# lunarlab-gatech/SLIDE_SLAM

Hardware: AMD Instinct MI355X
Metric: pose-graph updates/sec + ms/Gauss-Newton iter, 8-robot 10k-landmark graph (higher is better)
Workload: dtype f64

## Files before the change

slide_slam_amd/csrc/graph_dev.hpp:

```cpp
#pragma once
#include <stdint.h>

namespace sl {

enum { VT_POSE = 0, VT_POINT = 1, VT_CUBE = 2, VT_CYL = 3 };
enum { FT_BR = 2, FT_CUBE = 3, FT_CYL = 4 };

constexpr int NB = 64;

__host__ __device__ inline int lm_dim(int t) { return t == VT_POINT ? 3 : (t == VT_CUBE ? 9 : 7); }
__host__ __device__ inline int lf_rows(int t) { return t == FT_BR ? 3 : (t == FT_CUBE ? 9 : 7); }
__host__ __device__ inline int lf_jsize(int t) { return t == FT_BR ? 30 : (t == FT_CUBE ? 144 : 98); }
__host__ __device__ inline int lf_esize(int t) { return t == FT_BR ? 42 : (t == FT_CUBE ? 114 : 90); }

struct GraphDev {
  int P, L;
  double* pose_val;
  double* pose_delta;
  double* pose_est;
  int* lm_type;
  double* lm_val;
  double* lm_delta;
  double* lm_est;
  int n_prior;
  int* pr_pose; double* pr_z; double* pr_sigma;
  double* pr_r;
  int n_between;
  int* bt_i; int* bt_j; double* bt_z; double* bt_sigma;
  double* bt_r; double* bt_J0;
  int n_ghost;
  int* gh_pose; int* gh_slot; int* gh_first;
  double* gh_z; double* gh_sigma;
  double* gh_r; double* gh_J;
  int n_gslots; double* ghost_val; int* gslot_pose;
  int n_lf;
  int n_nbr;
  int* lf_type; int* lf_pose; int* lf_lm; int* lf_slot;
  int* lf_nbr;
  int64_t* lf_joff; int64_t* lf_eoff;
  double* br_z;
  double* cu_z; double* cu_sigma;
  double* cy_z;
  double* jbuf;
  double* ebuf;
  int* lm_ptr; int* lm_fids;
  int* pose_ptr; int* pose_fids;
  int* pose_lms;
  long long* pose_ed;
  int* pose_bt_ptr; int* pose_bt;
  unsigned* pose_adj; int adj_words;
  double* lm_Hinv;
  double* lm_g;
  double* lm_Hacc;
  double* lm_t;
  int n_slots;
  int* sh_lid;
  int* sh_owner;
  double* pose_H;
  double* pose_g;
  double* S;
  int ld;
  int T;
  double* Ld;
  double* Winv;
  double* yv;
  double* dp;
  int* chol_ctr;
  const int* prof;
  const int* first;
  int prof_ver;
  int schur_split;
  double* S0;
  int save_S0;
  double* pcg;
  const int* lm_slot;
  double* pcg_scal;
  double pcg_tol2;
  int arrow;
  int nbr;
  const int* lm_bord;
  const int* seg_tab;
  double* bord;
  int ldb;
  double* bord0;
  const int* pose_sep;
  int nsep;
  int nsep_dim;
  const int* gh_bord;
  const int* lm_first;
  int pose0;
  int col0;
  const int* sp_idx;
  const long long* sp_pairs;
  int sp_w;
  int* status;
  int chart;
  double relin_thr;
  double bearing_sigma, cyl_sigma, numdiff_delta;
};

struct RobustDev {
  double* bt_sigma0;
  double* bt_w; double* bt_s2;
  int* bt_kind;
  double* gh_sigma0;
  double* gh_w; double* gh_s2;
  int kind;
  int mask;
  double param;
};

struct ObsLossDev {
  double* lf_w; double* lf_s2;
  int kind;
  int mask;
  double param;
};

}
```

slide_slam_amd/csrc/kernels.hpp:

```cpp
#pragma once
#include <hip/hip_runtime.h>
#include <stdint.h>

#include "graph_dev.hpp"
#include "sl_math.hpp"

namespace sl {

void init_solver_kernels();
void launch_relin(const GraphDev& G, hipStream_t s);
void launch_linearize(const GraphDev& G, const ObsLossDev& O, hipStream_t s);
void launch_observation_weights(const GraphDev& G, const ObsLossDev& O, bool robust, int n, double* out2n, hipStream_t s);
void launch_observation_weights_batched(const GraphDev* d, const ObsLossDev* dO, bool robust, const int* off, const int* cnt, int n, double* out2n,
                                        hipStream_t s);
void launch_robust_reweight(const GraphDev& G, const RobustDev& R, hipStream_t s);
void launch_closure_weights(const GraphDev& G, const RobustDev& R, const int* idx, int n, double* out2n, hipStream_t s);
void launch_robust_reweight_batched(const GraphDev* d, const RobustDev* dR, const GraphDev* h, int n, hipStream_t s);
void launch_closure_weights_batched(const GraphDev* d, const RobustDev* dR, const int* ent2, int n, double* out2n, hipStream_t s);
void launch_landmark(const GraphDev& G, int mode, hipStream_t s);
void launch_pose(const GraphDev& G, hipStream_t s);
void launch_schur(const GraphDev& G, hipStream_t s);
void launch_backsub(const GraphDev& G, int mode, hipStream_t s);
void launch_shared_pack(const GraphDev& G, int what, double* buf, hipStream_t s);
void launch_shared_unpack(const GraphDev& G, int what, const double* buf, hipStream_t s);
// ... 192 lines not shown
  }
  return lo;
}
struct TriSeg { int tm0, td0, ntd; };
void launch_tri_match_seg(bool emit, const double* sd, const double* sx, const int* rowoff, const TriSeg* segs, int n_seg, int n_rows, double thr,
                          int* counts, const long long* offs, const long long* base, double* P1, double* P2, hipStream_t s);
void launch_seg_scan64(const int* cnt, const int* segoff, int n_seg, long long* out, long long* totals, hipStream_t s);
void launch_seg_scan_rowptr(const int* cnt, const int* segoff, int n_seg, int* rowptr, long long* totals, hipStream_t s);
struct ClqSolve {
  const int* rowptr; const int* col; const double* val; int n;
  const double* u0;
  double *u, *unew, *g, *gnew, *Mu, *Cu;
  double tol_u, tol_F, beta, eps;
  int maxin, maxol, maxls, rescale;
  double* out;
};
void launch_clq_solve_batch(const ClqSolve* d_jobs, int n_jobs, hipStream_t s);
bool launch_clq_solve_coop(const ClqSolve& A, double* priv, int* bar2, int n_wg, hipStream_t s);
void launch_clq_csr_count(const double* Mup, int n, int* rowcnt, hipStream_t s);
void launch_clq_csr_fill(const double* Mup, int n, const int* rowptr, int* col, double* val, hipStream_t s);
void launch_clq_solve(const int* rowptr, const int* col, const double* val, int n, const double* u0, double* work6n, double tol_u, double tol_F,
                      double beta, double eps, int maxin, int maxol, int maxls, int rescale, double* out4, hipStream_t s);
void launch_clipper_affinity(const double* D1, const double* D2, int dim, const int32_t* A, int m, double sigma, double eps,
                             double mindist, double affinityeps, double* M, hipStream_t s);
template <int DIM>
__device__ __forceinline__ double clipper_pair_score(int i0, int i1, int j0, int j1, const double* pi1, const double* pj1, const double* pi2,
                                                     const double* pj2, int dim, double sigma, double eps, double mindist, double affinityeps) {
  double out = 0.0;
  if (i0 != j0 && i1 != j1) {
    const int nd = DIM > 0 ? DIM : dim;
    double s1 = 0, s2 = 0;
    for (int k = 0; k < nd; ++k) {
      s1 += (pi1[k] - pj1[k]) * (pi1[k] - pj1[k]);
      s2 += (pi2[k] - pj2[k]) * (pi2[k] - pj2[k]);
    }
    const double l1 = sqrt(s1), l2 = sqrt(s2);
    if (!(mindist > 0 && (l1 < mindist || l2 < mindist))) {
      const double c = fabs(l1 - l2);
      const double scr = (c < eps) ? exp(-0.5 * c * c / (sigma * sigma)) : 0.0;
      if (scr > affinityeps) out = scr;
    }
  }
  return out;
}
void launch_affinity_gather(const double* D1, const double* D2, int dim, const int32_t* A, int m, double* P1, double* P2, hipStream_t s);
void launch_affinity_csr(bool emit, const double* D1, const double* D2, const double* P1, const double* P2, int dim, const int32_t* A, int m,
                         double sigma, double eps, double mindist, double affinityeps, int* rowcnt, const int* rowptr, int* col, double* val,
                         hipStream_t s);
void launch_affinity_csr_seg(bool emit, const double* P1, const double* P2, const int* aoff, int n_seg, int n_rows, double sigma, double eps,
                             double mindist, double affinityeps, int* rowcnt, const int* rowptr, const long long* nnz0, int* col, double* val,
                             hipStream_t s);
void launch_clq_pack_u(const double* work, const int* aoff, int n_seg, int n_rows, double* U, hipStream_t s);

constexpr int CLOSURE_PRE = 36;
struct ClosureScore { double gate, sigma, affinityeps, odom2[6]; };
__host__ __device__ __forceinline__ double closure_pair_score(const double* __restrict__ pre_i, const double* __restrict__ pre_j, const double* __restrict__ s2i,
                                                              const double* __restrict__ s2j, double legs, const ClosureScore& P) {
  const SE3 E = compose(compose(from12(pre_i), from12(pre_j + 12)), from12(pre_i + 24));
  double e[6];
  se3_log(E, e);
  double q = 0.0;
#pragma unroll
  for (int c = 0; c < 6; ++c) q += e[c] * e[c] / (s2i[c] + s2j[c] + legs * P.odom2[c]);
  const double d = sqrt(q);
  const double scr = d < P.gate ? exp(-0.5 * d * d / (P.sigma * P.sigma)) : 0.0;
  return scr > P.affinityeps ? scr : 0.0;
}
__host__ __device__ __forceinline__ void closure_prepare_one(const SE3& F, const SE3& T, const SE3& z, double* __restrict__ pre) {
  const SE3 U = compose(z, inverse(T));
  to12(U, pre);
  to12(inverse(compose(F, U)), pre + 12);
  to12(F, pre + 24);
}
void launch_closure_prepare(const double* fpose12, const double* tpose12, const int32_t* fslot, const int32_t* tslot, const double* z12, int n,
                            double* pre, hipStream_t s);
void launch_closure_csr_seg(bool emit, const double* pre, const double* sig2, const unsigned long long* idx2, const int* goff, int n_seg,
                            int n_rows, const ClosureScore& P, int* rowcnt, const int* rowptr, const long long* nnz0, int* col, double* val,
                            hipStream_t s);

constexpr int GATE_OUT = 43;
void launch_closure_gate_lin(const double* pose_est, const int32_t* fslot, const int32_t* tslot, const double* z12, const double* sigma6, int n,
                             int chart, const int* prow, double* B, int nT, double* r6, hipStream_t s);
void launch_pair_identity(const int32_t* aslot, const int32_t* bslot, int n, const int* prow, double* B, int nT, hipStream_t s);
struct JointPoseTab { const double* est[JSIG_ROBOTS_MAX]; const int* prow[JSIG_ROBOTS_MAX]; long long off[JSIG_ROBOTS_MAX]; int chart[JSIG_ROBOTS_MAX]; };
void launch_joint_closure_gate_lin(const JointPoseTab* tab, const int4* ends, const double* z12, const double* sigma6, int n, double* B,
                                   size_t ld, double* r6, hipStream_t s);
void launch_joint_pair_identity(const JointPoseTab* tab, const int4* ends, int n, double* B, size_t ld, hipStream_t s);
void launch_gram_sub(double* M, const double* Mneg, size_t n, hipStream_t s);
void launch_closure_gate_finish(const double* M, const double* r6, int n, double* out, int* flag, hipStream_t s);

constexpr int OBS_GATE_OUT = 91;
void launch_obs_gate_lin(const GraphDev& G, int type, const int32_t* pid, const int32_t* lid, const double* z15, const double* sg9, int n,
                         double* B, int nT, double* r9, double* G0, hipStream_t s);
void launch_joint_obs_gate_lin(const GraphDev* Gs, const JointPoseTab* tab, int type, const int4* ends, const long long* sep_row, const double* z15,
                               const double* sg9, int n, double* B, size_t ld, double* r9, double* G0, hipStream_t s);
void launch_obs_gate_finish(int m, const double* M, const double* G0, const double* r9, int n, double* out, int* flag, hipStream_t s);

}
```

slide_slam_amd/csrc/pcg_kernels.hip:

```cpp
#include <hip/hip_runtime.h>

#include "graph_dev.hpp"
#include "kernels.hpp"

namespace sl {

enum { PV_R = 0, PV_U = 1, PV_W = 2, PV_P = 3, PV_S = 4, PV_X = 5, PV_Y = 6, PV_COUNT = 7 };
__device__ __forceinline__ double* pvec(const GraphDev& G, int i) { return G.pcg + (size_t)i * G.T * NB; }

__global__ __launch_bounds__(256) void k_pcg_init(const GraphDev* __restrict__ Gs) {
  const GraphDev G = Gs[blockIdx.z];
  const int i = blockIdx.x * 256 + threadIdx.x, nT = G.T * NB;
  if (i >= nT) return;
  pvec(G, PV_R)[i] = i < 6 * G.P ? -G.pose_g[i] : 0.0;
  pvec(G, PV_U)[i] = G.dp[i];
  pvec(G, PV_X)[i] = 0.0;
  pvec(G, PV_P)[i] = 0.0;
  pvec(G, PV_S)[i] = 0.0;
  if (i < 8) G.pcg_scal[i] = 0.0;
}

struct PcgBufs { double* p[8]; };

__device__ __forceinline__ void pcg_tl_body(const GraphDev& G, const PcgBufs& B, int blk, int vec) {
  const int wave = threadIdx.x >> 6, lane = threadIdx.x & 63;
  const int sidx = blk * 4 + wave;
  if (sidx >= G.n_slots) return;
  double* out = B.p[blockIdx.z] + 9 * (size_t)sidx;
  const int l = G.sh_lid[sidx];
  if (l < 0) {
    if (lane < 9) out[lane] = 0.0;
    return;
  }
  const double* v = pvec(G, vec);
  const int D = lm_dim(G.lm_type[l]);
  double rhs[9];
#pragma unroll
  for (int k = 0; k < 9; ++k) rhs[k] = 0.0;
  for (int q = G.lm_ptr[l] + lane; q < G.lm_ptr[l + 1]; q += 64) {
    const int f = G.lm_fids[q];
    const double* E = G.ebuf + G.lf_eoff[f];
    const double* d = v + 6 * (size_t)G.lf_pose[f];
    double dd[6];
#pragma unroll
    for (int a = 0; a < 6; ++a) dd[a] = d[a];
#pragma unroll
    for (int k = 0; k < 9; ++k) {
      if (k < D) {
        double s = 0.0;
#pragma unroll
        for (int a = 0; a < 6; ++a) s += E[a * D + k] * dd[a];
        rhs[k] += s;
      }
    }
  }
#pragma unroll
  for (int k = 0; k < 9; ++k) {
#pragma unroll
    for (int m = 32; m >= 1; m >>= 1) rhs[k] += __shfl_xor(rhs[k], m);
  }
  if (lane == 0) {
#pragma unroll
    for (int k = 0; k < 9; ++k) {
      G.lm_t[9 * (size_t)l + k] = rhs[k];
      out[k] = rhs[k];
    }
  }
}

__device__ __forceinline__ void pcg_symv_body(const GraphDev& G, int bi, int vin, int vout, int in_lds) {
  if (bi >= G.T) return;
  extern __shared__ double xs_lds[];
  __shared__ double red[4][NB];
  __shared__ double redt[NB][5];
  const int tid = threadIdx.x, row = tid & 63, cp = tid >> 6;
  const double* x = pvec(G, vin);
  const double* S0 = G.S0;
  const int ld = G.ld, nT = G.T * NB;
  if (in_lds) {
    for (int i = tid; i < nT; i += 256) xs_lds[i] = x[i];
    __syncthreads();
  }
  const double* xs = in_lds ? xs_lds : x;
  double acc = 0.0;
  {
    double ta[16], tb[16];
    const double* tp0 = S0 + (size_t)(16 * cp) * ld + (size_t)bi * NB + row;
    const int jf = G.first ? G.first[bi] : 0;
    if (jf < bi) {
      const double* tp = tp0 + (size_t)(jf * NB) * ld;
#pragma unroll
      for (int r = 0; r < 16; ++r) ta[r] = tp[(size_t)r * ld];
    }
    for (int j = jf; j < bi; j += 2) {
      if (j + 1 < bi) {
        const double* tp = tp0 + (size_t)((j + 1) * NB) * ld;
#pragma unroll
        for (int r = 0; r < 16; ++r) tb[r] = tp[(size_t)r * ld];
      }
      {
        const double* xj = xs + j * NB + 16 * cp;
#pragma unroll
        for (int r = 0; r < 16; ++r) acc += ta[r] * xj[r];
      }
      if (j + 2 < bi) {
        const double* tp = tp0 + (size_t)((j + 2) * NB) * ld;
#pragma unroll
        for (int r = 0; r < 16; ++r) ta[r] = tp[(size_t)r * ld];
      }
      if (j + 1 < bi) {
        const double* xj = xs + (j + 1) * NB + 16 * cp;
#pragma unroll
        for (int r = 0; r < 16; ++r) acc += tb[r] * xj[r];
      }
    }
  }
  {
    const double* tp = S0 + (size_t)(bi * NB) * ld + (size_t)bi * NB;
    const double* xj = xs + bi * NB;
#pragma unroll
    for (int r = 0; r < 16; ++r) {
      const int c = 16 * cp + r;
      const double v = c <= row ? tp[(size_t)c * ld + row] : tp[(size_t)row * ld + c];
      acc += v * xj[c];
    }
  }
  red[cp][row] = acc;
  const int col = tid >> 2, part = tid & 3;
  double acct = 0.0;
  {
    double ta[16], tb[16];
    const double* tp0 = S0 + (size_t)(bi * NB + col) * ld + 16 * part;
    const int j0 = bi + 1, T = G.prof ? G.prof[bi] + 1 : G.T;
    if (j0 < T) {
#pragma unroll
      for (int r = 0; r < 16; ++r) ta[r] = tp0[(size_t)j0 * NB + r];
    }
    for (int j = j0; j < T; j += 2) {
      if (j + 1 < T) {
#pragma unroll
        for (int r = 0; r < 16; ++r) tb[r] = tp0[(size_t)(j + 1) * NB + r];
      }
      {
        const double* xj = xs + j * NB + 16 * part;
#pragma unroll
        for (int r = 0; r < 16; ++r) acct += ta[r] * xj[r];
      }
      if (j + 2 < T) {
#pragma unroll
        for (int r = 0; r < 16; ++r) ta[r] = tp0[(size_t)(j + 2) * NB + r];
      }
      if (j + 1 < T) {
        const double* xj = xs + (j + 1) * NB + 16 * part;
#pragma unroll
        for (int r = 0; r < 16; ++r) acct += tb[r] * xj[r];
      }
    }
  }
  redt[col][part] = acct;
  __syncthreads();
  if (tid < NB) {
    const double a = (red[0][tid] + red[1][tid]) + (red[2][tid] + red[3][tid]);
    const double b = (redt[tid][0] + redt[tid][1]) + (redt[tid][2] + redt[tid][3]);
    pvec(G, vout)[(size_t)bi * NB + tid] = a + b;
  }
}

__global__ __launch_bounds__(256) void k_pcg_tl_symv(const GraphDev* __restrict__ Gs, PcgBufs B, int vec, int vout, int n_row_blocks, int in_lds) {
  const GraphDev G = Gs[blockIdx.z];
  if ((int)blockIdx.x < n_row_blocks) pcg_symv_body(G, blockIdx.x, vec, vout, in_lds);
  else pcg_tl_body(G, B, (int)blockIdx.x - n_row_blocks, vec);
}

__global__ __launch_bounds__(256) void k_pcg_cross(const GraphDev* __restrict__ Gs, PcgBufs B, int vout, int nsum) {
  const GraphDev G = Gs[blockIdx.z];
  const int wave = threadIdx.x >> 6, lane = threadIdx.x & 63;
  const int p = blockIdx.x * 4 + wave;
  if (p >= G.P) return;
  double y[6];
#pragma unroll
  for (int a = 0; a < 6; ++a) y[a] = 0.0;
  for (int q = G.pose_ptr[p] + lane; q < G.pose_ptr[p + 1]; q += 64) {
    const int l = G.pose_lms[q];
    const int sl = G.lm_slot[l];
    if (sl < 0) continue;
    const long long ed = G.pose_ed[q];
    const int D = (int)(ed & 15);
    const double* town = G.lm_t + 9 * (size_t)l;
    double cc[9];
#pragma unroll
    for (int k = 0; k < 9; ++k) cc[k] = 0.0;
    if (nsum > 1) {
#pragma unroll
      for (int k = 0; k < 9; ++k) {
        if (k < D) {
          double t[8];
#pragma unroll
          for (int r = 0; r < 8; ++r) t[r] = r < nsum ? B.p[r][9 * (size_t)sl + k] : 0.0;
          double acc = 0.0;
#pragma unroll
          for (int r = 0; r < 8; ++r)
            if (r < nsum) acc += t[r];
          cc[k] = acc;
        }
      }
    } else {
      const double* tsum = B.p[blockIdx.z] + 9 * (size_t)sl;
#pragma unroll
      for (int k = 0; k < 9; ++k) cc[k] = k < D ? tsum[k] : 0.0;
    }
#pragma unroll
    for (int k = 0; k < 9; ++k) cc[k] = k < D ? cc[k] - town[k] : 0.0;
    const double* F = G.ebuf + (ed >> 4) + 6 * D;
#pragma unroll
    for (int a = 0; a < 6; ++a) {
      double s = 0.0;
#pragma unroll
      for (int k = 0; k < 9; ++k)
        if (k < D) s += F[a * D + k] * cc[k];
      y[a] += s;
    }
  }
#pragma unroll
  for (int a = 0; a < 6; ++a) {
#pragma unroll
    for (int m = 32; m >= 1; m >>= 1) y[a] += __shfl_xor(y[a], m);
  }
  if (lane < 6) {
    double v = 0.0;
#pragma unroll
    for (int a = 0; a < 6; ++a) v = lane == a ? y[a] : v;
    pvec(G, vout)[6 * (size_t)p + lane] -= v;
  }
}

__global__ __launch_bounds__(256) void k_pcg_dots(const GraphDev* __restrict__ Gs, PcgBufs B) {
  const GraphDev G = Gs[blockIdx.z];
  __shared__ double sh[2][256];
  const int tid = threadIdx.x, nT = G.T * NB;
  const double* r = pvec(G, PV_R);
  const double* u = pvec(G, PV_U);
  const double* w = pvec(G, PV_W);
  double a = 0.0, b = 0.0;
  for (int i = tid; i < nT; i += 256) {
    const double ui = u[i];
    a += r[i] * ui;
    b += w[i] * ui;
  }
  sh[0][tid] = a;
  sh[1][tid] = b;
  __syncthreads();
  for (int st = 128; st > 0; st >>= 1) {
    if (tid < st) { sh[0][tid] += sh[0][tid + st]; sh[1][tid] += sh[1][tid + st]; }
// ... 105 lines not shown
```

slide_slam_amd/csrc/solver_kernels.hip:

```cpp
#include <hip/hip_runtime.h>
#include <algorithm>
#include <cstring>

#include "graph_dev.hpp"
#include "kernels.hpp"
#include "sl_math.hpp"

namespace sl {

struct BufPtrs { double* p[8]; };

__device__ inline void pose_retract12(const double* in12, const double* d6, int chart, double* out12) {
  to12(retract(from12(in12), d6, chart), out12);
}
__device__ inline void lm_retract(int type, const double* in, const double* d, int chart, double* out) {
  if (type == VT_POINT) {
    out[0] = in[0] + d[0]; out[1] = in[1] + d[1]; out[2] = in[2] + d[2];
  } else if (type == VT_CUBE) {
    pose_retract12(in, d, chart, out);
    out[12] = in[12] + d[6]; out[13] = in[13] + d[7]; out[14] = in[14] + d[8];
  } else {
    out[3] = in[3] + d[0]; out[4] = in[4] + d[1]; out[5] = in[5] + d[2];
    out[0] = in[0] + d[3]; out[1] = in[1] + d[4]; out[2] = in[2] + d[5];
    out[6] = in[6] + d[6];
// ... 214 lines not shown
#pragma unroll
        for (int k = 0; k < 3; ++k) { s += Dm[3 * r + k] * Q.a[3 * k + j]; u += Dm[3 * r + k] * X.R.a[3 * j + k]; }
        Jp[6 * r + j] = sc(s * w);
        Jp[6 * r + 3 + j] = sc(-Dm[3 * r + j] * w);
        Jl[3 * r + j] = sc(u * w);
      }
  } else if (type == FT_CUBE) {
    const double* z = G.cu_z + 15 * (size_t)slot;
    const double* sg = G.cu_sigma + 9 * (size_t)slot;
    const SE3 C = from12(lv);
    double dX[6], dC[6], cs[3];
#pragma unroll
    for (int k = 0; k < 6; ++k) { dX[k] = (col == k) ? d : 0.0; dC[k] = (col == 6 + k) ? d : 0.0; }
#pragma unroll
    for (int k = 0; k < 3; ++k) cs[k] = lv[12 + k] + ((col == 12 + k) ? d : 0.0);
    double e[9];
    cube_err(retract(X, dX, G.chart), retract(C, dC, G.chart), cs, z, e);
    if constexpr (ROBUST) {
      double s2 = 0.0;
#pragma unroll
      for (int i = 0; i < 9; ++i) { const double q = __shfl(e[i], 30, 32) * (1.0 / sg[i]); s2 += q * q; }
      sq = obs_loss_scale(O, FT_CUBE, f, s2, j == 30);
    }
#pragma unroll
    for (int i = 0; i < 9; ++i) {
      const double hx = __shfl(e[i], 30, 32), eo = __shfl_xor(e[i], 1, 32), w = 1.0 / sg[i];
      if (j == 30) out[i] = sc(hx * w);
      if ((j & 1) == 0 && col < 15) {
        const double v = sc(((e[i] - hx) - (eo - hx)) * fac * w);
        if (col < 6) out[9 + 6 * i + col] = v;
        else out[63 + 9 * i + col - 6] = v;
      }
    }
  } else {
    const double* z = G.cy_z + 7 * (size_t)slot;
    const double w = 1.0 / G.cyl_sigma;
    const int jl = col - 6;
    const int vi = jl < 0 ? -1 : (jl < 3 ? jl + 3 : (jl < 6 ? jl - 3 : (jl == 6 ? 6 : -1)));
    double dX[6], q[7];
#pragma unroll
    for (int k = 0; k < 6; ++k) dX[k] = (col == k) ? d : 0.0;
#pragma unroll
    for (int k = 0; k < 7; ++k) q[k] = lv[k] + ((vi == k) ? d : 0.0);
    double e[7];
    cyl_err(retract(X, dX, G.chart), q, z, e);
    if constexpr (ROBUST) {
      double s2 = 0.0;
#pragma unroll
      for (int i = 0; i < 7; ++i) { const double q = __shfl(e[i], 30, 32) * w; s2 += q * q; }
      sq = obs_loss_scale(O, FT_CYL, f, s2, j == 30);
    }
#pragma unroll
    for (int i = 0; i < 7; ++i) {
      const double hx = __shfl(e[i], 30, 32), eo = __shfl_xor(e[i], 1, 32);
      if (j == 30) out[i] = sc(hx * w);
      if ((j & 1) == 0 && col < 13) {
        const double v = sc(((e[i] - hx) - (eo - hx)) * fac * w);
        if (col < 6) out[7 + 6 * i + col] = v;
        else out[49 + 7 * i + jl] = v;
      }
    }
  }
}
__global__ __launch_bounds__(256) void k_lin_lf(GraphDev G, int nb0, int nb1) {
  if ((int)blockIdx.x < nb0) k_lin_pose_factors_body(G, blockIdx.x * 256 + threadIdx.x);
  else k_lin_lf_body<false>(G, ObsLossDev{}, nb1, (int)blockIdx.x - nb0);
}
__global__ __launch_bounds__(256) void k_lin_lf_robust(GraphDev G, ObsLossDev O, int nb0, int nb1) {
  if ((int)blockIdx.x < nb0) k_lin_pose_factors_body(G, blockIdx.x * 256 + threadIdx.x);
  else k_lin_lf_body<true>(G, O, nb1, (int)blockIdx.x - nb0);
}
__global__ __launch_bounds__(256) void k_lin_lf_b(const GraphDev* __restrict__ Gs, int nb0, int nb1) {
  if ((int)blockIdx.x < nb0) k_lin_pose_factors_body(Gs[blockIdx.z], blockIdx.x * 256 + threadIdx.x);
  else k_lin_lf_body<false>(Gs[blockIdx.z], ObsLossDev{}, nb1, (int)blockIdx.x - nb0);
}
__global__ __launch_bounds__(256) void k_lin_lf_robust_b(const GraphDev* __restrict__ Gs, const ObsLossDev* __restrict__ Os, int nb0, int nb1) {
  if ((int)blockIdx.x < nb0) k_lin_pose_factors_body(Gs[blockIdx.z], blockIdx.x * 256 + threadIdx.x);
  else k_lin_lf_body<true>(Gs[blockIdx.z], Os[blockIdx.z], nb1, (int)blockIdx.x - nb0);
}

__shared__ double lm_hs[4][96];
constexpr int LM_RED_MAX = 24;
__shared__ double lm_red[4][54 * LM_RED_MAX];

template <int D, int MODE>
__device__ inline void landmark_wave(const GraphDev& G, int l, int lane) {
  constexpr int NH = D * (D + 1) / 2;
  double h[NH], g[D];
#pragma unroll
  for (int i = 0; i < NH; ++i) h[i] = 0.0;
#pragma unroll
  for (int i = 0; i < D; ++i) g[i] = 0.0;
  const int f0 = G.lm_ptr[l], nf = G.lm_ptr[l + 1] - f0;
  double* acc = G.lm_Hacc + 54 * (size_t)l;
  if (MODE == 2) {
#pragma unroll
    for (int i = 0; i < NH; ++i) h[i] = acc[i];
#pragma unroll
    for (int i = 0; i < D; ++i) g[i] = acc[45 + i];
  }
  for (int q = lane; MODE != 2 && q < nf; q += 64) {
    const int f = G.lm_fids[f0 + q];
    const double* rec = G.jbuf + G.lf_joff[f];
    const double* Jl = rec + D + 6 * D;
#pragma unroll
    for (int k = 0; k < D; ++k) {
      double row[D];
#pragma unroll
      for (int a = 0; a < D; ++a) row[a] = Jl[D * k + a];
      const double rk = rec[k];
#pragma unroll
      for (int a = 0; a < D; ++a) {
        g[a] += row[a] * rk;
#pragma unroll
        for (int c = 0; c <= a; ++c) h[a * (a + 1) / 2 + c] += row[a] * row[c];
      }
    }
  }
  if (MODE != 2) {
    if (MODE == 3) {
      double* red = lm_red[threadIdx.x >> 6];
      const int nl = nf < 64 ? nf : 64;
      double tot = 0.0;
      for (int base = 0; base < nl; base += LM_RED_MAX) {
        const int cnt = nl - base < LM_RED_MAX ? nl - base : LM_RED_MAX;
        if (lane >= base && lane < base + cnt) {
#pragma unroll
          for (int i = 0; i < NH; ++i) red[i * LM_RED_MAX + lane - base] = h[i];
#pragma unroll
          for (int i = 0; i < D; ++i) red[(NH + i) * LM_RED_MAX + lane - base] = g[i];
        }
        __builtin_amdgcn_wave_barrier();
        __builtin_amdgcn_s_waitcnt(0xc07f);
        if (lane < NH + D)
          for (int q = 0; q < cnt; ++q) tot += red[lane * LM_RED_MAX + q];
        __builtin_amdgcn_wave_barrier();
        __builtin_amdgcn_s_waitcnt(0xc07f);
      }
      if (lane < NH + D) red[lane] = tot;
      __builtin_amdgcn_wave_barrier();
      __builtin_amdgcn_s_waitcnt(0xc07f);
#pragma unroll
      for (int i = 0; i < NH; ++i) h[i] = red[i];
#pragma unroll
      for (int i = 0; i < D; ++i) g[i] = red[NH + i];
    } else {
#pragma unroll
      for (int off = 32; off > 0; off >>= 1) {
#pragma unroll
        for (int i = 0; i < NH; ++i) h[i] += __shfl_xor(h[i], off);
#pragma unroll
        for (int i = 0; i < D; ++i) g[i] += __shfl_xor(g[i], off);
      }
    }
  }
  if (MODE == 1 || MODE == 3) {
    if (lane == 0) {
#pragma unroll
      for (int i = 0; i < NH; ++i) acc[i] = h[i];
#pragma unroll
      for (int i = 0; i < D; ++i) acc[45 + i] = g[i];
    }
    if (MODE == 1) return;
  }
  double* Hinv = G.lm_Hinv + 81 * (size_t)l;
  double* gout = G.lm_g + 9 * (size_t)l;
// ... 1 lines not shown
#pragma unroll
    for (int a = 0; a < D; ++a) gout[a] = g[a];
  }
  const bool sep = (MODE == 2 || MODE == 3) && G.arrow && G.lm_slot && G.lm_slot[l] >= 0;
  if (nf == 0 && (MODE == 0 || MODE == 3)) {
    if (lane == 0) {
#pragma unroll
      for (int i = 0; i < D * D; ++i) Hinv[i] = 0.0;
    }
    return;
  }
  double Cm[D][D];
  bool ok = true;
#pragma unroll
  for (int j = 0; j < D; ++j) {
    double s = h[j * (j + 1) / 2 + j];
#pragma unroll
    for (int k = 0; k < j; ++k) s -= Cm[j][k] * Cm[j][k];
    if (!(s > 0.0)) { ok = false; s = 1.0; }
    const double dj = sqrt(s);
    Cm[j][j] = dj;
#pragma unroll
    for (int i = j + 1; i < D; ++i) {
      double t = h[i * (i + 1) / 2 + j];
#pragma unroll
      for (int k = 0; k < j; ++k) t -= Cm[i][k] * Cm[j][k];
      Cm[i][j] = t / dj;
    }
  }
  if (!ok && !sep && lane == 0) atomicOr(&G.status[0], 1);
  double Ci[D][D];
#pragma unroll
  for (int c = 0; c < D; ++c) {
    Ci[c][c] = 1.0 / Cm[c][c];
#pragma unroll
    for (int i = c + 1; i < D; ++i) {
      double s = 0.0;
#pragma unroll
      for (int k = c; k < i; ++k) s -= Cm[i][k] * Ci[k][c];
      Ci[i][c] = s / Cm[i][i];
    }
  }
  double Hi[D][D];
#pragma unroll
  for (int a = 0; a < D; ++a)
#pragma unroll
    for (int c = 0; c <= a; ++c) {
      double s = 0.0;
#pragma unroll
      for (int k = a; k < D; ++k) s += Ci[k][a] * Ci[k][c];
      if (sep) s = 0.0;
      Hi[a][c] = s;
      Hi[c][a] = s;
    }
  if (lane == 0) {
#pragma unroll
    for (int a = 0; a < D; ++a)
#pragma unroll
      for (int c = 0; c < D; ++c) Hinv[a * D + c] = Hi[a][c];
  }
  double* hs = lm_hs[threadIdx.x >> 6];
  if (lane == 0) {
#pragma unroll
    for (int a = 0; a < D; ++a) {
#pragma unroll
      for (int c = 0; c < D; ++c) hs[a * D + c] = Hi[a][c];
      hs[81 + a] = g[a];
    }
  }
  __builtin_amdgcn_wave_barrier();
  __builtin_amdgcn_s_waitcnt(0xc07f);
  for (int it = lane; it < 6 * nf; it += 64) {
    const int q = it / 6, a = it - 6 * q;
    const int f = G.lm_fids[f0 + q];
    const double* rec = G.jbuf + G.lf_joff[f];
    const double* Jp = rec + D;
    const double* Jl = rec + D + 6 * D;
    double* E = G.ebuf + G.lf_eoff[f];
    double* F = E + 6 * D;
    double* u = F + 6 * D;
    double Ea[D];
#pragma unroll
    for (int c = 0; c < D; ++c) Ea[c] = 0.0;
#pragma unroll
    for (int k = 0; k < D; ++k) {
      const double jp = Jp[6 * k + a];
#pragma unroll
      for (int c = 0; c < D; ++c) Ea[c] += jp * Jl[D * k + c];
    }
#pragma unroll
    for (int c = 0; c < D; ++c) E[a * D + c] = Ea[c];
    double ua = 0.0;
#pragma unroll
    for (int c = 0; c < D; ++c) {
      double sF = 0.0;
#pragma unroll
      for (int k = 0; k < D; ++k) sF += Ea[k] * hs[k * D + c];
      F[a * D + c] = sF;
      ua += sF * hs[81 + c];
    }
    u[a] = ua;
  }
}

template <int MODE>
__device__ __forceinline__ void k_landmark_body(const GraphDev& G) {
  const int l = blockIdx.x * 4 + (threadIdx.x >> 6);
  if (l >= G.L) return;
  const int lane = threadIdx.x & 63;
  if (G.pose0 > 0) {
    bool any = false;
    for (int q = G.lm_ptr[l] + lane; q < G.lm_ptr[l + 1]; q += 64) any = any || G.lf_pose[G.lm_fids[q]] >= G.pose0;
    if (!__ballot(any)) return;
  }
  const int type = G.lm_type[l];
  if (type == VT_POINT) landmark_wave<3, MODE>(G, l, lane);
  else if (type == VT_CUBE) landmark_wave<9, MODE>(G, l, lane);
  else landmark_wave<7, MODE>(G, l, lane);
}
template <int MODE>
__global__ __launch_bounds__(256) void k_landmark(GraphDev G) { k_landmark_body<MODE>(G); }
template <int MODE>
__global__ __launch_bounds__(256) void k_landmark_b(const GraphDev* __restrict__ Gs) {
  const GraphDev G = Gs[blockIdx.z];
  k_landmark_body<MODE>(G);
}

__device__ __forceinline__ void k_pose_body(const GraphDev& G) {
  __shared__ double part[4][27][65];
  const int wave = threadIdx.x >> 6, lane = threadIdx.x & 63;
  const int p = blockIdx.x * 4 + wave;
  if (p >= G.P || p < G.pose0) return;
  double H[21], g[6];
#pragma unroll
  for (int i = 0; i < 21; ++i) H[i] = 0.0;
#pragma unroll
  for (int i = 0; i < 6; ++i) g[i] = 0.0;
  const int nbt = G.pose_bt_ptr[p + 1] - G.pose_bt_ptr[p];
  const int nlf = G.pose_ptr[p + 1] - G.pose_ptr[p];
  const int nun = G.n_prior + G.n_ghost;
  for (int e = lane; e < nun + nbt + nlf; e += 64) {
    if (e < G.n_prior) {
      if (G.pr_pose[e] != p) continue;
#pragma unroll
      for (int k = 0; k < 6; ++k) {
        const double w = 1.0 / G.pr_sigma[6 * e + k];
        H[k * (k + 1) / 2 + k] += w * w;
        g[k] += w * G.pr_r[6 * e + k];
      }
    } else if (e < nun) {
      const int q = e - G.n_prior;
      if (G.gh_pose[q] != p || (G.arrow && G.gh_bord)) continue;
      const double* J = G.gh_J + 36 * (size_t)q;
      const double* r = G.gh_r + 6 * (size_t)q;
#pragma unroll
      for (int k = 0; k < 6; ++k) {
        double jr[6];
#pragma unroll
        for (int a = 0; a < 6; ++a) jr[a] = J[6 * k + a];
        const double rk = r[k];
#pragma unroll
        for (int a = 0; a < 6; ++a) {
          g[a] += jr[a] * rk;
#pragma unroll
          for (int c = 0; c <= a; ++c) H[a * (a + 1) / 2 + c] += jr[a] * jr[c];
        }
      }
    } else if (e < nun + nbt) {
      const int ent = G.pose_bt[G.pose_bt_ptr[p] + e - nun];
      const int b = ent >> 1, role = ent & 1;
      const double* r = G.bt_r + 6 * (size_t)b;
// ... 126 lines not shown
  for (int q = tid; q < nb; q += 256) {
    const int l = G.pose_lms[b0 + q];
    if (q == 0 || G.pose_lms[b0 + q - 1] != l) schur_slot[l] = (short)q;
    if (q < SCHUR_PJ_CAP) { pj_lm[q] = l; pj_ed[q] = G.pose_ed[b0 + q]; }
  }
  __syncthreads();
  const int sub = tid & 7;
  int p_end = G.P;
  if (G.prof) {
    const int rows = (G.prof[(6 * pj + 5) / NB] + 1) * NB;
    p_end = min(G.P, (rows + 5) / 6);
  }
  for (int pi0 = pj + 32 * yb; pi0 < p_end; pi0 += 32 * (int)gridDim.y) {
    const int nval = 6 * min(32, G.P - pi0);
    double* Sb = G.S + (size_t)(6 * pj) * G.ld + 6 * (size_t)pi0;
    double* S0b = G.S0 + (size_t)(6 * pj) * G.ld + 6 * (size_t)pi0;
    const int w = pi0 >> 5, sh = pi0 & 31;
    const unsigned m = sh ? ((adj[w] >> sh) | (adj[w + 1] << (32 - sh))) : adj[w];
    if (m == 0u) {
      for (int e = tid; e < 6 * 192; e += 256) {
        const int c = e / 192, r = e % 192;
        if (r < nval && 6 * pj + c >= G.col0) {
          Sb[(size_t)c * G.ld + r] = 0.0;
          if (G.save_S0) S0b[(size_t)c * G.ld + r] = 0.0;
        }
      }
      continue;
    }
  const int pi = pi0 + (tid >> 3);
  const bool live = pi < G.P && ((m >> (tid >> 3)) & 1u);
  double acc[36];
#pragma unroll
  for (int k = 0; k < 36; ++k) acc[k] = 0.0;
  if (live) {
    if (sub == 0) {
      if (pi == pj) {
#pragma unroll
        for (int k = 0; k < 36; ++k) acc[k] = G.pose_H[36 * (size_t)pi + k];
      } else {
        for (int q = G.pose_bt_ptr[pi]; q < G.pose_bt_ptr[pi + 1]; ++q) {
          const int ent = G.pose_bt[q];
          const int b = ent >> 1, role = ent & 1;
          const int other = role ? G.bt_i[b] : G.bt_j[b];
          if (other != pj) continue;
          const double* J = G.bt_J0 + 36 * (size_t)b;
          if (role == 1) {
#pragma unroll
            for (int a = 0; a < 6; ++a) {
              const double w = 1.0 / G.bt_sigma[6 * b + a];
#pragma unroll
              for (int c = 0; c < 6; ++c) acc[6 * a + c] += w * J[6 * a + c];
            }
          } else {
#pragma unroll
            for (int c = 0; c < 6; ++c) {
              const double w = 1.0 / G.bt_sigma[6 * b + c];
#pragma unroll
              for (int a = 0; a < 6; ++a) acc[6 * a + c] += J[6 * c + a] * w;
            }
          }
        }
      }
    }
    const int a0 = G.pose_ptr[pi], a1 = G.pose_ptr[pi + 1];
    for (int x0 = a0 + sub; x0 < a1; x0 += 24) {
      int sl[3];
      long long ed[3];
#pragma unroll
      for (int u = 0; u < 3; ++u) {
        const int x = x0 + 8 * u;
        sl[u] = -1;
        ed[u] = 0;
        if (x < a1) {
          const int l = G.pose_lms[x];
          ed[u] = G.pose_ed[x];
          sl[u] = schur_slot[l];
        }
      }
#pragma unroll
      for (int u = 0; u < 3; ++u) {
        if (sl[u] < 0) continue;
        const int D = (int)(ed[u] & 15);
        const double* F = G.ebuf + (ed[u] >> 4) + 6 * D;
        const int l = (sl[u] < SCHUR_PJ_CAP) ? pj_lm[sl[u]] : G.pose_lms[b0 + sl[u]];
        for (int y = sl[u]; y < nb; ++y) {
          const int ly = (y < SCHUR_PJ_CAP) ? pj_lm[y] : G.pose_lms[b0 + y];
          if (ly != l) break;
          const long long edy = (y < SCHUR_PJ_CAP) ? pj_ed[y] : G.pose_ed[b0 + y];
          const double* E = G.ebuf + (edy >> 4);
          if (D == 3) {
            double e[18];
#pragma unroll
            for (int k = 0; k < 18; ++k) e[k] = E[k];
#pragma unroll
            for (int a = 0; a < 6; ++a) {
              const double f0 = F[3 * a], f1 = F[3 * a + 1], f2 = F[3 * a + 2];
#pragma unroll
              for (int c = 0; c < 6; ++c) acc[6 * a + c] -= f0 * e[3 * c] + f1 * e[3 * c + 1] + f2 * e[3 * c + 2];
            }
          } else {
            for (int k = 0; k < D; ++k) {
              double fk[6], ek[6];
#pragma unroll
              for (int a = 0; a < 6; ++a) { fk[a] = F[a * D + k]; ek[a] = E[a * D + k]; }
#pragma unroll
              for (int a = 0; a < 6; ++a)
#pragma unroll
                for (int c = 0; c < 6; ++c) acc[6 * a + c] -= fk[a] * ek[c];
            }
          }
        }
      }
    }
  }
#pragma unroll
  for (int k = 0; k < 36; ++k) {
    acc[k] += dpp_f64<0xB1>(acc[k]);
    acc[k] += dpp_f64<0x4E>(acc[k]);
    acc[k] += dpp_f64<0x141>(acc[k]);
  }
#pragma unroll
  for (int c = 0; c < 6; ++c)
    if (sub == c) {
#pragma unroll
      for (int a = 0; a < 6; ++a) schur_tile[c][6 * (tid >> 3) + a] = acc[6 * a + c];
    }
  __syncthreads();
  for (int e = tid; e < 6 * 192; e += 256) {
    const int c = e / 192, r = e % 192;
    if (r < nval && 6 * pj + c >= G.col0) {
      Sb[(size_t)c * G.ld + r] = schur_tile[c][r];
      if (G.save_S0) S0b[(size_t)c * G.ld + r] = schur_tile[c][r];
    }
  }
  __syncthreads();
  }
}
__device__ __forceinline__ void k_pad_rhs_body(const GraphDev& G, int bid);
__device__ __forceinline__ void k_border_fill_body(const GraphDev& G, int bid);
__device__ __forceinline__ void k_border_fill_lam_body(const GraphDev& G, int bid);
__global__ __launch_bounds__(256) void k_schur(GraphDev G, int p_first) {
  const int x = (int)blockIdx.x + p_first;
  if (x >= G.P) {
    if (blockIdx.y == 0) k_pad_rhs_body(G, x - G.P);
    return;
  }
  k_schur_body(G, x, blockIdx.y);
}
__global__ __launch_bounds__(256) void k_schur_b(const GraphDev* __restrict__ Gs) {
  const GraphDev G = Gs[blockIdx.z];
  k_schur_body(G, blockIdx.x, blockIdx.y);
}
constexpr int SCHUR_KC = 2;

template <int KC>
__device__ __forceinline__ void schur_pair_cols(const char* __restrict__ ebase, unsigned fb, unsigned eb, int D, int k0, double (&acc)[36]) {
  double fk[KC][6], ek[KC][6];
#pragma unroll
  for (int u = 0; u < KC; ++u)
#pragma unroll
    for (int a = 0; a < 6; ++a) {
      const unsigned o = (unsigned)(a * D + k0) * 8u;
      fk[u][a] = *reinterpret_cast<const double*>(ebase + (fb + o) + 8 * u);
      ek[u][a] = *reinterpret_cast<const double*>(ebase + (eb + o) + 8 * u);
    }
#pragma unroll
  for (int u = 0; u < KC; ++u)
#pragma unroll
    for (int a = 0; a < 6; ++a)
#pragma unroll
      for (int c = 0; c < 6; ++c) acc[6 * a + c] = fma(-fk[u][a], ek[u][c], acc[6 * a + c]);
}
__device__ __forceinline__ void k_schur_listed_body(const GraphDev& G, int pj, int yb) {
  __shared__ double schur_tile[6][192];
  if (pj >= G.P) return;
  if (6 * pj + 5 < G.col0) return;
  const int tid = threadIdx.x;
  const int sub = tid & 7;
  const unsigned* __restrict__ adj = G.pose_adj + (size_t)pj * G.adj_words;
  int p_end = G.P;
  if (G.prof) {
    const int rows = (G.prof[(6 * pj + 5) / NB] + 1) * NB;
    p_end = min(G.P, (rows + 5) / 6);
  }
  for (int pi0 = pj + 32 * yb; pi0 < p_end; pi0 += 32 * (int)gridDim.y) {
    const int nval = 6 * min(32, G.P - pi0);
    double* Sb = G.S + (size_t)(6 * pj) * G.ld + 6 * (size_t)pi0;
    double* S0b = G.S0 + (size_t)(6 * pj) * G.ld + 6 * (size_t)pi0;
    const int w = pi0 >> 5, sh = pi0 & 31;
    const unsigned aw0 = adj[w], aw1 = adj[w + 1];
    const unsigned m = sh ? ((aw0 >> sh) | (aw1 << (32 - sh))) : aw0;
    if (m == 0u) {
      for (int e = tid; e < 6 * 192; e += 256) {
        const int c = e / 192, r = e % 192;
        if (r < nval && 6 * pj + c >= G.col0) {
          Sb[(size_t)c * G.ld + r] = 0.0;
          if (G.save_S0) S0b[(size_t)c * G.ld + r] = 0.0;
        }
      }
      continue;
    }
    const int pi = pi0 + (tid >> 3);
    const bool live = pi < G.P && ((m >> (tid >> 3)) & 1u);
    double acc[36];
#pragma unroll
    for (int k = 0; k < 36; ++k) acc[k] = 0.0;
    if (live) {
      const int2 qc = *reinterpret_cast<const int2*>(G.sp_idx + 2 * ((size_t)pj * G.sp_w + (pi - pj)));
      if (sub == 0) {
        if (pi == pj) {
#pragma unroll
          for (int k = 0; k < 36; ++k) acc[k] = G.pose_H[36 * (size_t)pi + k];
        } else {
          for (int q = G.pose_bt_ptr[pi]; q < G.pose_bt_ptr[pi + 1]; ++q) {
            const int ent = G.pose_bt[q];
            const int b = ent >> 1, role = ent & 1;
            const int other = role ? G.bt_i[b] : G.bt_j[b];
            if (other != pj) continue;
            const double* J = G.bt_J0 + 36 * (size_t)b;
            if (role == 1) {
#pragma unroll
              for (int a = 0; a < 6; ++a) {
                const double w = 1.0 / G.bt_sigma[6 * b + a];
#pragma unroll
                for (int c = 0; c < 6; ++c) acc[6 * a + c] += w * J[6 * a + c];
              }
            } else {
#pragma unroll
              for (int c = 0; c < 6; ++c) {
                const double w = 1.0 / G.bt_sigma[6 * b + c];
#pragma unroll
                for (int a = 0; a < 6; ++a) acc[6 * a + c] += J[6 * c + a] * w;
              }
            }
          }
        }
      }
      const int q0 = qc.x, q1 = qc.x + qc.y;
      const longlong2* __restrict__ prs = reinterpret_cast<const longlong2*>(G.sp_pairs);
      const char* __restrict__ ebase = reinterpret_cast<const char*>(G.ebuf);
      for (int x0 = q0 + sub; x0 < q1; x0 += 24) {
        const longlong2 z2 = longlong2{0, 0};
        const longlong2 e0 = prs[x0];
        const longlong2 e1 = x0 + 8 < q1 ? prs[x0 + 8] : z2;
        const longlong2 e2 = x0 + 16 < q1 ? prs[x0 + 16] : z2;
#pragma unroll 1
        for (int u = 0; u < 3 && x0 + 8 * u < q1; ++u) {
          const longlong2 e = u == 0 ? e0 : (u == 1 ? e1 : e2);
          const int D = (int)(e.x & 15);
          const unsigned fb = ((unsigned)(e.x >> 4) + 6u * D) * 8u, eb = (unsigned)(e.y >> 4) * 8u;
          int k = 0;
#pragma unroll 1
          for (; k + SCHUR_KC <= D; k += SCHUR_KC) schur_pair_cols<SCHUR_KC>(ebase, fb, eb, D, k, acc);
#pragma unroll 1
          for (; k < D; ++k) schur_pair_cols<1>(ebase, fb, eb, D, k, acc);
        }
      }
    }
#pragma unroll
    for (int k = 0; k < 36; ++k) {
      acc[k] += dpp_f64<0xB1>(acc[k]);
      acc[k] += dpp_f64<0x4E>(acc[k]);
      acc[k] += dpp_f64<0x141>(acc[k]);
    }
#pragma unroll
    for (int c = 0; c < 6; ++c)
      if (sub == c) {
#pragma unroll
        for (int a = 0; a < 6; ++a) schur_tile[c][6 * (tid >> 3) + a] = acc[6 * a + c];
      }
    __syncthreads();
    for (int e = tid; e < 6 * 192; e += 256) {
      const int c = e / 192, r = e % 192;
      if (r < nval && 6 * pj + c >= G.col0) {
        Sb[(size_t)c * G.ld + r] = schur_tile[c][r];
        if (G.save_S0) S0b[(size_t)c * G.ld + r] = schur_tile[c][r];
      }
    }
    __syncthreads();
  }
}
__global__ __launch_bounds__(256) void k_schur_lb(const GraphDev* __restrict__ Gs, int xcd, int np, int npad, int nfill, int nlam) {
  int x = blockIdx.x, y = blockIdx.y, z = blockIdx.z;
  if (xcd) {
    const long long total = (long long)gridDim.x * gridDim.y * gridDim.z;
    const long long lin = x + (long long)gridDim.x * (y + (long long)gridDim.y * z);
    const int r = (int)(lin % 8);
    long long l2 = lin / 8;
    for (int i = 0; i < r; ++i) l2 += (total - i + 7) / 8;
    x = (int)(l2 % gridDim.x);
    y = (int)((l2 / gridDim.x) % gridDim.y);
    z = (int)(l2 / ((long long)gridDim.x * gridDim.y));
  }
  const GraphDev G = Gs[z];
  if (x >= np) {
    int r = (x - np) * (int)gridDim.y + y;
    if (r < npad) { k_pad_rhs_body(G, r); return; }
    r -= npad;
    if (r < nfill) { k_border_fill_body(G, r); return; }
    r -= nfill;
    if (r < nlam) k_border_fill_lam_body(G, r);
    return;
  }
  k_schur_listed_body(G, x, y);
}

struct ScatterSeg { unsigned long long dst; unsigned off, bytes; };
__global__ __launch_bounds__(256) void k_scatter(const unsigned char* __restrict__ stage, unsigned desc_off) {
  const ScatterSeg sg = reinterpret_cast<const ScatterSeg*>(stage + desc_off)[blockIdx.x];
  const unsigned* src = reinterpret_cast<const unsigned*>(stage + sg.off);
  unsigned* dst = reinterpret_cast<unsigned*>(sg.dst);
  const unsigned n = sg.bytes >> 2;
  for (unsigned i = blockIdx.y * 256 + threadIdx.x; i < n; i += 256 * gridDim.y) dst[i] = src[i];
}
struct SumBcastArgs { int n; double* buf[8]; };
__global__ __launch_bounds__(256) void k_sum_bcast(SumBcastArgs A, int count) {
  const int i = blockIdx.x * 256 + threadIdx.x;
  if (i >= count) return;
  double s = 0.0;
  for (int r = 0; r < A.n; ++r) s += A.buf[r][i];
  for (int r = 0; r < A.n; ++r) A.buf[r][i] = s;
}
void launch_sum_bcast(double* const* bufs, int n, int count, hipStream_t s) {
// ... 1163 lines not shown
```

Before: 3994.

## Tag device pointers as global address space, prefetch landmark Jacobian rows, specialize symv

Wraps every device pointer in the graph views with a global-address-space wrapper in the device pass, so the compiler can emit global loads instead of flat loads. Layout stays identical to the host and is checked with static asserts. The landmark E-block product now software-pipelines its Jacobian row loads in double-buffered pairs, separated by scheduling barriers. The PCG symv body is templated on whether its input vector sits in LDS, removing a runtime branch. Risks include higher register pressure from the prefetch buffers and a large cross-file type change that all pointer uses must tolerate.

```diff
diff --git a/slide_slam_amd/csrc/graph_dev.hpp b/slide_slam_amd/csrc/graph_dev.hpp
--- a/slide_slam_amd/csrc/graph_dev.hpp
+++ b/slide_slam_amd/csrc/graph_dev.hpp
@@ -1,5 +1,7 @@
 #pragma once
 #include <stdint.h>
+
+#include <type_traits>
 
 namespace sl {
 
@@ -13,108 +15,131 @@
 __host__ __device__ inline int lf_jsize(int t) { return t == FT_BR ? 30 : (t == FT_CUBE ? 144 : 98); }
 __host__ __device__ inline int lf_esize(int t) { return t == FT_BR ? 42 : (t == FT_CUBE ? 114 : 90); }
 
+#if defined(__HIP_DEVICE_COMPILE__)
+template <typename T>
+struct GlobalPtr {
+  __attribute__((address_space(1))) T* p;
+  GlobalPtr() = default;
+  __host__ __device__ __forceinline__ GlobalPtr(T* q) : p((__attribute__((address_space(1))) T*)q) {}
+  __host__ __device__ __forceinline__ operator T*() const { return (T*)p; }
+  template <typename U>
+  __host__ __device__ __forceinline__ GlobalPtr(const GlobalPtr<U>& o) : p(o.p) {}
+};
+static_assert(sizeof(GlobalPtr<double>) == sizeof(double*) && alignof(GlobalPtr<double>) == alignof(double*), "the host copies the views as plain pointers");
+#define SL_GPTR(T) GlobalPtr<T>
+template <typename T>
+__device__ __forceinline__ __attribute__((address_space(1))) T* global_of(const GlobalPtr<T>& g) { return g.p; }
+#else
+#define SL_GPTR(T) T*
+template <typename T>
+__host__ __device__ inline T* global_of(T* p) { return p; }
+#endif
+
 struct GraphDev {
   int P, L;
-  double* pose_val;
-  double* pose_delta;
-  double* pose_est;
-  int* lm_type;
-  double* lm_val;
-  double* lm_delta;
-  double* lm_est;
+  SL_GPTR(double) pose_val;
+  SL_GPTR(double) pose_delta;
+  SL_GPTR(double) pose_est;
+  SL_GPTR(int) lm_type;
+  SL_GPTR(double) lm_val;
+  SL_GPTR(double) lm_delta;
+  SL_GPTR(double) lm_est;
   int n_prior;
-  int* pr_pose; double* pr_z; double* pr_sigma;
-  double* pr_r;
+  SL_GPTR(int) pr_pose; SL_GPTR(double) pr_z; SL_GPTR(double) pr_sigma;
+  SL_GPTR(double) pr_r;
   int n_between;
-  int* bt_i; int* bt_j; double* bt_z; double* bt_sigma;
-  double* bt_r; double* bt_J0;
+  SL_GPTR(int) bt_i; SL_GPTR(int) bt_j; SL_GPTR(double) bt_z; SL_GPTR(double) bt_sigma;
+  SL_GPTR(double) bt_r; SL_GPTR(double) bt_J0;
   int n_ghost;
-  int* gh_pose; int* gh_slot; int* gh_first;
-  double* gh_z; double* gh_sigma;
-  double* gh_r; double* gh_J;
-  int n_gslots; double* ghost_val; int* gslot_pose;
+  SL_GPTR(int) gh_pose; SL_GPTR(int) gh_slot; SL_GPTR(int) gh_first;
+  SL_GPTR(double) gh_z; SL_GPTR(double) gh_sigma;
+  SL_GPTR(double) gh_r; SL_GPTR(double) gh_J;
+  int n_gslots; SL_GPTR(double) ghost_val; SL_GPTR(int) gslot_pose;
   int n_lf;
   int n_nbr;
-  int* lf_type; int* lf_pose; int* lf_lm; int* lf_slot;
-  int* lf_nbr;
-  int64_t* lf_joff; int64_t* lf_eoff;
-  double* br_z;
-  double* cu_z; double* cu_sigma;
-  double* cy_z;
-  double* jbuf;
-  double* ebuf;
-  int* lm_ptr; int* lm_fids;
-  int* pose_ptr; int* pose_fids;
-  int* pose_lms;
-  long long* pose_ed;
-  int* pose_bt_ptr; int* pose_bt;
-  unsigned* pose_adj; int adj_words;
-  double* lm_Hinv;
-  double* lm_g;
-  double* lm_Hacc;
-  double* lm_t;
+  SL_GPTR(int) lf_type; SL_GPTR(int) lf_pose; SL_GPTR(int) lf_lm; SL_GPTR(int) lf_slot;
+  SL_GPTR(int) lf_nbr;
+  SL_GPTR(int64_t) lf_joff; SL_GPTR(int64_t) lf_eoff;
+  SL_GPTR(double) br_z;
+  SL_GPTR(double) cu_z; SL_GPTR(double) cu_sigma;
+  SL_GPTR(double) cy_z;
+  SL_GPTR(double) jbuf;
+  SL_GPTR(double) ebuf;
+  SL_GPTR(int) lm_ptr; SL_GPTR(int) lm_fids;
+  SL_GPTR(int) pose_ptr; SL_GPTR(int) pose_fids;
+  SL_GPTR(int) pose_lms;
+  SL_GPTR(long long) pose_ed;
+  SL_GPTR(int) pose_bt_ptr; SL_GPTR(int) pose_bt;
+  SL_GPTR(unsigned) pose_adj; int adj_words;
+  SL_GPTR(double) lm_Hinv;
+  SL_GPTR(double) lm_g;
+  SL_GPTR(double) lm_Hacc;
+  SL_GPTR(double) lm_t;
   int n_slots;
-  int* sh_lid;
-  int* sh_owner;
-  double* pose_H;
-  double* pose_g;
-  double* S;
+  SL_GPTR(int) sh_lid;
+  SL_GPTR(int) sh_owner;
+  SL_GPTR(double) pose_H;
+  SL_GPTR(double) pose_g;
+  SL_GPTR(double) S;
   int ld;
   int T;
-  double* Ld;
-  double* Winv;
-  double* yv;
-  double* dp;
-  int* chol_ctr;
-  const int* prof;
-  const int* first;
+  SL_GPTR(double) Ld;
+  SL_GPTR(double) Winv;
+  SL_GPTR(double) yv;
+  SL_GPTR(double) dp;
+  SL_GPTR(int) chol_ctr;
+  SL_GPTR(const int) prof;
+  SL_GPTR(const int) first;
   int prof_ver;
   int schur_split;
-  double* S0;
+  SL_GPTR(double) S0;
   int save_S0;
-  double* pcg;
-  const int* lm_slot;
-  double* pcg_scal;
+  SL_GPTR(double) pcg;
+  SL_GPTR(const int) lm_slot;
+  SL_GPTR(double) pcg_scal;
   double pcg_tol2;
   int arrow;
   int nbr;
-  const int* lm_bord;
-  const int* seg_tab;
-  double* bord;
+  SL_GPTR(const int) lm_bord;
+  SL_GPTR(const int) seg_tab;
+  SL_GPTR(double) bord;
   int ldb;
-  double* bord0;
-  const int* pose_sep;
+  SL_GPTR(double) bord0;
+  SL_GPTR(const int) pose_sep;
   int nsep;
   int nsep_dim;
-  const int* gh_bord;
-  const int* lm_first;
+  SL_GPTR(const int) gh_bord;
+  SL_GPTR(const int) lm_first;
   int pose0;
   int col0;
-  const int* sp_idx;
-  const long long* sp_pairs;
+  SL_GPTR(const int) sp_idx;
+  SL_GPTR(const long long) sp_pairs;
   int sp_w;
-  int* status;
+  SL_GPTR(int) status;
   int chart;
   double relin_thr;
   double bearing_sigma, cyl_sigma, numdiff_delta;
 };
 
 struct RobustDev {
-  double* bt_sigma0;
-  double* bt_w; double* bt_s2;
-  int* bt_kind;
-  double* gh_sigma0;
-  double* gh_w; double* gh_s2;
+  SL_GPTR(double) bt_sigma0;
+  SL_GPTR(double) bt_w; SL_GPTR(double) bt_s2;
+  SL_GPTR(int) bt_kind;
+  SL_GPTR(double) gh_sigma0;
+  SL_GPTR(double) gh_w; SL_GPTR(double) gh_s2;
   int kind;
   int mask;
   double param;
 };
 
 struct ObsLossDev {
-  double* lf_w; double* lf_s2;
+  SL_GPTR(double) lf_w; SL_GPTR(double) lf_s2;
   int kind;
   int mask;
   double param;
 };
 
+static_assert(sizeof(GraphDev) == 800 && sizeof(RobustDev) == 72 && sizeof(ObsLossDev) == 32, "the views' layout is the same in both passes");
+static_assert(std::is_trivially_copyable<GraphDev>::value && std::is_standard_layout<GraphDev>::value, "GraphDev is copied bytewise and passed by value");
+
 }
diff --git a/slide_slam_amd/csrc/kernels.hpp b/slide_slam_amd/csrc/kernels.hpp
--- a/slide_slam_amd/csrc/kernels.hpp
+++ b/slide_slam_amd/csrc/kernels.hpp
@@ -298,7 +298,8 @@
 void launch_closure_gate_lin(const double* pose_est, const int32_t* fslot, const int32_t* tslot, const double* z12, const double* sigma6, int n,
                              int chart, const int* prow, double* B, int nT, double* r6, hipStream_t s);
 void launch_pair_identity(const int32_t* aslot, const int32_t* bslot, int n, const int* prow, double* B, int nT, hipStream_t s);
-struct JointPoseTab { const double* est[JSIG_ROBOTS_MAX]; const int* prow[JSIG_ROBOTS_MAX]; long long off[JSIG_ROBOTS_MAX]; int chart[JSIG_ROBOTS_MAX]; };
+struct JointPoseTab { SL_GPTR(const double) est[JSIG_ROBOTS_MAX]; SL_GPTR(const int) prow[JSIG_ROBOTS_MAX]; long long off[JSIG_ROBOTS_MAX]; int chart[JSIG_ROBOTS_MAX]; };
+static_assert(sizeof(JointPoseTab) == (2 * sizeof(void*) + sizeof(long long) + sizeof(int)) * JSIG_ROBOTS_MAX, "host and device passes see the same bytes");
 void launch_joint_closure_gate_lin(const JointPoseTab* tab, const int4* ends, const double* z12, const double* sigma6, int n, double* B,
                                    size_t ld, double* r6, hipStream_t s);
 void launch_joint_pair_identity(const JointPoseTab* tab, const int4* ends, int n, double* B, size_t ld, hipStream_t s);
diff --git a/slide_slam_amd/csrc/pcg_kernels.hip b/slide_slam_amd/csrc/pcg_kernels.hip
--- a/slide_slam_amd/csrc/pcg_kernels.hip
+++ b/slide_slam_amd/csrc/pcg_kernels.hip
@@ -68,7 +68,8 @@
   }
 }
 
-__device__ __forceinline__ void pcg_symv_body(const GraphDev& G, int bi, int vin, int vout, int in_lds) {
+template <bool IN_LDS>
+__device__ __forceinline__ void pcg_symv_body(const GraphDev& G, int bi, int vin, int vout) {
   if (bi >= G.T) return;
   extern __shared__ double xs_lds[];
   __shared__ double red[4][NB];
@@ -77,11 +78,11 @@
   const double* x = pvec(G, vin);
   const double* S0 = G.S0;
   const int ld = G.ld, nT = G.T * NB;
-  if (in_lds) {
+  if (IN_LDS) {
     for (int i = tid; i < nT; i += 256) xs_lds[i] = x[i];
     __syncthreads();
   }
-  const double* xs = in_lds ? xs_lds : x;
+  const double* xs = IN_LDS ? xs_lds : x;
   double acc = 0.0;
   {
     double ta[16], tb[16];
@@ -168,7 +169,10 @@
 
 __global__ __launch_bounds__(256) void k_pcg_tl_symv(const GraphDev* __restrict__ Gs, PcgBufs B, int vec, int vout, int n_row_blocks, int in_lds) {
   const GraphDev G = Gs[blockIdx.z];
-  if ((int)blockIdx.x < n_row_blocks) pcg_symv_body(G, blockIdx.x, vec, vout, in_lds);
+  if ((int)blockIdx.x < n_row_blocks) {
+    if (in_lds) pcg_symv_body<true>(G, blockIdx.x, vec, vout);
+    else pcg_symv_body<false>(G, blockIdx.x, vec, vout);
+  }
   else pcg_tl_body(G, B, (int)blockIdx.x - n_row_blocks, vec);
 }
 
diff --git a/slide_slam_amd/csrc/solver_kernels.hip b/slide_slam_amd/csrc/solver_kernels.hip
--- a/slide_slam_amd/csrc/solver_kernels.hip
+++ b/slide_slam_amd/csrc/solver_kernels.hip
@@ -320,6 +320,7 @@
 __shared__ double lm_hs[4][96];
 constexpr int LM_RED_MAX = 24;
 __shared__ double lm_red[4][54 * LM_RED_MAX];
+constexpr int LM_KR = 2;
 
 template <int D, int MODE>
 __device__ inline void landmark_wave(const GraphDev& G, int l, int lane) {
@@ -487,11 +488,33 @@
     double Ea[D];
 #pragma unroll
     for (int c = 0; c < D; ++c) Ea[c] = 0.0;
-#pragma unroll
-    for (int k = 0; k < D; ++k) {
-      const double jp = Jp[6 * k + a];
-#pragma unroll
-      for (int c = 0; c < D; ++c) Ea[c] += jp * Jl[D * k + c];
+    constexpr int NG = (D + LM_KR - 1) / LM_KR;
+    double jp[2][LM_KR], jl[2][LM_KR][D];
+    auto load_rows = [&](int gq, int b) {
+#pragma unroll
+      for (int u = 0; u < LM_KR; ++u) {
+        const int k = gq * LM_KR + u;
+        if (k < D) {
+          jp[b][u] = Jp[6 * k + a];
+#pragma unroll
+          for (int c = 0; c < D; ++c) jl[b][u][c] = Jl[D * k + c];
+        }
+      }
+    };
+    load_rows(0, 0);
+#pragma unroll
+    for (int gq = 0; gq < NG; ++gq) {
+      if (gq + 1 < NG) load_rows(gq + 1, (gq + 1) & 1);
+      __builtin_amdgcn_sched_barrier(0);
+#pragma unroll
+      for (int u = 0; u < LM_KR; ++u) {
+        const int k = gq * LM_KR + u;
+        if (k < D) {
+#pragma unroll
+          for (int c = 0; c < D; ++c) Ea[c] += jp[gq & 1][u] * jl[gq & 1][u][c];
+        }
+      }
+      __builtin_amdgcn_sched_barrier(0);
     }
 #pragma unroll
     for (int c = 0; c < D; ++c) E[a * D + c] = Ea[c];
@@ -784,11 +807,11 @@
         if (sl[u] < 0) continue;
         const int D = (int)(ed[u] & 15);
         const double* F = G.ebuf + (ed[u] >> 4) + 6 * D;
-        const int l = (sl[u] < SCHUR_PJ_CAP) ? pj_lm[sl[u]] : G.pose_lms[b0 + sl[u]];
+        const int l = (sl[u] < SCHUR_PJ_CAP) ? pj_lm[sl[u]] : global_of(G.pose_lms)[b0 + sl[u]];
         for (int y = sl[u]; y < nb; ++y) {
-          const int ly = (y < SCHUR_PJ_CAP) ? pj_lm[y] : G.pose_lms[b0 + y];
+          const int ly = (y < SCHUR_PJ_CAP) ? pj_lm[y] : global_of(G.pose_lms)[b0 + y];
           if (ly != l) break;
-          const long long edy = (y < SCHUR_PJ_CAP) ? pj_ed[y] : G.pose_ed[b0 + y];
+          const long long edy = (y < SCHUR_PJ_CAP) ? pj_ed[y] : global_of(G.pose_ed)[b0 + y];
           const double* E = G.ebuf + (edy >> 4);
           if (D == 3) {
             double e[18];
@@ -939,8 +962,8 @@
         }
       }
       const int q0 = qc.x, q1 = qc.x + qc.y;
-      const longlong2* __restrict__ prs = reinterpret_cast<const longlong2*>(G.sp_pairs);
-      const char* __restrict__ ebase = reinterpret_cast<const char*>(G.ebuf);
+      const longlong2* __restrict__ prs = reinterpret_cast<const longlong2*>(static_cast<const long long*>(G.sp_pairs));
+      const char* __restrict__ ebase = reinterpret_cast<const char*>(static_cast<double*>(G.ebuf));
       for (int x0 = q0 + sub; x0 < q1; x0 += 24) {
         const longlong2 z2 = longlong2{0, 0};
         const longlong2 e0 = prs[x0];
```

Result: faster. 4142 (median of 6 runs) (+3.7%).
